# santi-pdp/segan_pytorch

Measured on AMD Instinct MI355X. Metric: 16384-sample waveform chunks/sec (GAN step), higher is better.
Workload: dtype f32

## Files before the change

segan_pytorch_amd/csrc/segan_conv.hip:

```cpp
#include "segan_conv_shared.h"

template <int MB, int NB, int WM, int U>
struct TileGeom {
  static constexpr int S = 32 / U;
  static constexpr int WN = 4 / WM;
  static constexpr int NI = MB / (32 * WM);
  static constexpr int NJ = NB / (32 * WN);
  static constexpr int NPT = MB / S;
};

struct TileWork {
  int tile, c0, c1;
  bool partial;
  int piece;
};

struct TileIter {
  int tileA;
  long unit, unit_end;
  int first_tile;
  __device__ __forceinline__ void init(const CorrArgs& a, int nch) {
    tileA = blockIdx.x;
    unit = (long)blockIdx.x * a.sk_units;
    unit_end = min(unit + (long)a.sk_units, a.sk_total);
// ... 293 lines not shown
            }
          }
        } else {
#pragma unroll
          for (int i = 0; i < NI; ++i) {
            const int rloc = 32 * (wm * NI + i) + (e & 3) + 8 * (e >> 2) + 4 * h;
            const int r = rloc / NPT;
            const int n = n0 + rloc % NPT;
            if (n >= a.Nout) continue;
            float v = acc[i][j][e] + (a.bias ? a.bias[n] : 0.0f);
            if (a.act == SEGAN_ACT_TANH) v = tanhf(v);
            const int P = S * q + r;
            int ii = P - a.o_padL;
            const size_t rowoff = (size_t)col_b[j] * a.Nout + n;
            if (ii >= 0 && ii < a.Lout) {
              if (a.o_roll != 0) {
                ii -= a.o_roll;
                if (ii < 0) ii += a.Lout;
                if (ii >= a.Lout) ii -= a.Lout;
              }
              a.out0[rowoff * (size_t)a.Lout + ii] = v;
            } else if (a.halo != nullptr) {
              if (ii < 0) a.halo[rowoff * hl + P] = v;
              else if (ii - a.Lout < a.o_padR) a.halo[rowoff * hl + a.o_padL + (ii - a.Lout)] = v;
            }
          }
        }
      }
    }
  }
}

template <int MB, bool OUT_HI>
__device__ __forceinline__ bool tile_is_dead(const CorrArgs& a, int m0) {
  if (OUT_HI) return false;
  if (a.out0 == nullptr && m0 + MB <= a.OC0) return true;
  if (a.out1 == nullptr && m0 >= a.OC0) return true;
  return false;
}

template <int MB, int U, int KC, int NI, int NJ, bool SHIFT, int FMODE = 0, int ZP = -1, int NPT = 32>
__device__ __forceinline__ void corr_mma_chunk(const float* Wl, const float* Il, int RLs,
                                               const int (&aoff)[NI], const int (&boff)[NJ],
                                               const int (&rsh)[NI], f32x16 (&acc)[NI][NJ],
                                               float (&b30)[NJ], int h, const int (&aoffx)[NI],
                                               const int (&boffx)[NJ]) {
  static_assert(FMODE == 0 || (!SHIFT && ZP < 0), "the pair trick of the F form has no row shifts");
  constexpr int NBI = SHIFT ? NI : 1;
  constexpr int CVC = KC / U;
  constexpr bool ZT = ZP >= 0 && CVC >= 2;
  typedef const volatile __attribute__((address_space(3))) float* ldsp;
  auto special = [](int i) { return ZT && (32 * i) / NPT == ZP; };
  auto skipped = [&](int i, int s) { return special(i) && ((2 * s) % U) == 0; };
  float av0[NI], av1[NI], bv0[NBI][NJ], bv1[NBI][NJ];
  auto read_step = [&](int s, float (&av)[NI], float (&bv)[NBI][NJ]) {
    const int kk = 2 * s;
    const int c = kk / U, u = kk % U;
    ldsp wr = (ldsp)(Wl + kk * MB);
    ldsp ir = (ldsp)(Il + c * RLs + u);
#pragma unroll
    for (int i = 0; i < NI; ++i)
      if (!skipped(i, s)) av[i] = wr[aoff[i]];
#pragma unroll
    for (int i = 0; i < NBI; ++i)
#pragma unroll
      for (int j = 0; j < NJ; ++j)
        if (!(SHIFT && skipped(i, s))) bv[i][j] = ir[boff[j] + (SHIFT ? rsh[i] : 0)];
  };
  constexpr int NS = FMODE == 1 ? KC / 2 - 1 : KC / 2;
  auto mma_step = [&](int s, const float (&av)[NI], float (&bv)[NBI][NJ]) {
    if (FMODE == 2 && s == NS - 1) {
#pragma unroll
      for (int j = 0; j < NJ; ++j) bv[0][j] = h ? b30[j] : bv[0][j];
    }
#pragma unroll
    for (int i = 0; i < NI; ++i)
#pragma unroll
      for (int j = 0; j < NJ; ++j)
        if (!skipped(i, s))
          acc[i][j] = __builtin_amdgcn_mfma_f32_32x32x2f32(av[i], bv[SHIFT ? i : 0][j], acc[i][j],
                                                           0, 0, 0);
  };
  if (FMODE == 1) {
    ldsp ir = (ldsp)(Il + (CVC - 1) * RLs + (U - 2));
#pragma unroll
    for (int j = 0; j < NJ; ++j) b30[j] = ir[boff[j] - h];
  }
  float avx[ZT ? CVC / 2 : 1][NI], bvx[ZT ? CVC / 2 : 1][NBI][NJ];
  if (ZT) {
#pragma unroll
    for (int p = 0; p < CVC / 2; ++p) {
      ldsp wr = (ldsp)(Wl + (2 * p * U + 1) * MB);
      ldsp ir = (ldsp)(Il + 2 * p * RLs + 1);
#pragma unroll
      for (int i = 0; i < NI; ++i)
        if (special(i)) avx[p][i] = wr[aoffx[i]];
#pragma unroll
      for (int i = 0; i < NBI; ++i)
#pragma unroll
        for (int j = 0; j < NJ; ++j)
          if (!SHIFT || special(i)) bvx[p][i][j] = ir[boffx[j] + (SHIFT ? rsh[i] : 0)];
    }
  }
  float av2[NI], bv2[NBI][NJ];
  read_step(0, av0, bv0);
  read_step(1, av1, bv1);
  if (ZT) {
    __builtin_amdgcn_sched_barrier(0);
#pragma unroll
    for (int p = 0; p < CVC / 2; ++p)
#pragma unroll
      for (int i = 0; i < NI; ++i)
#pragma unroll
        for (int j = 0; j < NJ; ++j)
          if (special(i))
            acc[i][j] = __builtin_amdgcn_mfma_f32_32x32x2f32(avx[p][i], bvx[p][SHIFT ? i : 0][j],
                                                             acc[i][j], 0, 0, 0);
  }
#pragma unroll
  for (int s = 0; s < NS; s += 3) {
    if (s + 2 < NS) read_step(s + 2, av2, bv2);
    __builtin_amdgcn_sched_barrier(0);
    mma_step(s, av0, bv0);
    __builtin_amdgcn_sched_barrier(0);
    if (s + 3 < NS) read_step(s + 3, av0, bv0);
    __builtin_amdgcn_sched_barrier(0);
    if (s + 1 < NS) mma_step(s + 1, av1, bv1);
    __builtin_amdgcn_sched_barrier(0);
    if (s + 4 < NS) read_step(s + 4, av1, bv1);
    __builtin_amdgcn_sched_barrier(0);
    if (s + 2 < NS) mma_step(s + 2, av2, bv2);
    __builtin_amdgcn_sched_barrier(0);
  }
}

template <int MB, int NB, int WM, int U, bool IN_HI, bool OUT_HI, bool SHIFT, int MAXPOS, int KC>
__global__ __launch_bounds__(256, 2) void corr_kernel(const CorrArgs a) {
  using G = TileGeom<MB, NB, WM, U>;
  constexpr int S = G::S, WN = G::WN, NI = G::NI, NJ = G::NJ, NPT = G::NPT;
  constexpr int SI = IN_HI ? S : 1;
  constexpr int CV = KC / U;
  static_assert(!OUT_HI || NPT % 32 == 0, "T-form tiles hold whole 32-row phase blocks");

  extern __shared__ __attribute__((aligned(16))) float smem[];
  const int RLs = a.RLs;
  float* Wl0 = smem;
  float* Il0 = smem + 2 * KC * MB;

  const int tid = threadIdx.x;
  const int lane = tid & 63;
  const int wave = __builtin_amdgcn_readfirstlane(tid >> 6);
  const int wm = wave / WN, wn = wave % WN;
  const int l31 = lane & 31, h = lane >> 5;

  const int nch = (a.Ktot + KC - 1) / KC;
  TileIter it;
  it.init(a, nch);
  TileWork tw;
  while (it.next(a, nch, tw)) {
  const int c0 = tw.c0, c1 = tw.c1;
  const int rowtile = a.rt0 + tw.tile / a.ncoltiles;
  const int coltile = tw.tile % a.ncoltiles;
  const int m0 = rowtile * MB;
  const int n0 = rowtile * NPT;
  if (tile_is_dead<MB, OUT_HI>(a, m0)) continue;
  const ColTile ct = make_coltile(coltile * NB, a.Tcols, NB);

  int pos_off[MAXPOS][SI];
  unsigned pos_ok[MAXPOS];
  int pos_bo0[MAXPOS], pos_bo1[MAXPOS];
#pragma unroll
  for (int pp = 0; pp < MAXPOS; ++pp) {
    const int j = tid + 256 * pp;
    pos_ok[pp] = 0u;
    pos_bo0[pp] = 0;
    pos_bo1[pp] = 0;
#pragma unroll
    for (int r = 0; r < SI; ++r) pos_off[pp][r] = 0;
    if (j < RLs) {
      int s, tau;
      lds_pos_decode(ct, j, a.Tcols, a.H, s, tau);
      const int b = ct.b0 + s;
      if (b < a.B) {
        pos_bo0[pp] = b * a.in.C0 * a.Lin;
        pos_bo1[pp] = b * a.in.C1 * a.Lin;
        const int wq = tau + a.win_start;
        if (IN_HI) {
#pragma unroll
          for (int r = 0; r < SI; ++r) {
            const int idx = segan_hi_index(S * wq + r, a.Lin, a.padL, a.mode, a.roll);
            if (idx >= 0) { pos_off[pp][r] = idx; pos_ok[pp] |= 1u << r; }
          }
        } else if (wq >= 0 && wq < a.Lin) {
          pos_off[pp][0] = wq;
          pos_ok[pp] = 1u;
        }
      }
    }
  }

  int aoff[NI], boff[NJ], rsh[NI];
#pragma unroll
  for (int i = 0; i < NI; ++i) {
    const int rloc = 32 * (wm * NI + i);
    aoff[i] = h * MB + rloc + l31;
    rsh[i] = SHIFT ? a.rowshift[rloc / NPT] : 0;
  }
  int col_b[NJ], col_t[NJ];
  lane_columns<NB, WN, NJ>(a, ct, wn, l31, h, col_b, col_t, boff);

  f32x16 acc[NI][NJ];
#pragma unroll
  for (int i = 0; i < NI; ++i)
#pragma unroll
    for (int j = 0; j < NJ; ++j)
#pragma unroll
      for (int e = 0; e < 16; ++e) acc[i][j][e] = 0.0f;

  constexpr int F4R = MB / 4;
  constexpr int RPP = 256 / F4R;
  constexpr int NPASS = KC / RPP;
  f32x4 wreg[NPASS];
  float ireg[CV][MAXPOS];
  const int wrow = tid / F4R, wc4 = tid % F4R;
  const int wgcol = OUT_HI ? ((4 * wc4) / NPT) * a.NP + n0 + (4 * wc4) % NPT : m0 + 4 * wc4;
  const float* wbase = a.wp + (size_t)wrow * a.RP + wgcol;

  auto load_chunk = [&](int ch) {
    const float* wsrc = wbase + (size_t)(ch * KC) * a.RP;
#pragma unroll
    for (int p = 0; p < NPASS; ++p)
      wreg[p] = *reinterpret_cast<const f32x4*>(wsrc + (size_t)(RPP * p) * a.RP);
#pragma unroll
    for (int c = 0; c < CV; ++c) {
      int cv = ch * CV + c;
      cv = cv < a.Cv ? cv : 0;
      const int n = IN_HI ? cv / S : cv;
      const int r = IN_HI ? c % S : 0;
      const bool seg1 = n >= a.in.C0;
      const float* rowp = seg1 ? a.in.p1 + (size_t)(n - a.in.C0) * a.Lin
                               : a.in.p0 + (size_t)n * a.Lin;
#pragma unroll
      for (int pp = 0; pp < MAXPOS; ++pp)
        ireg[c][pp] = rowp[(seg1 ? pos_bo1[pp] : pos_bo0[pp]) + pos_off[pp][r]];
    }
  };
  auto store_chunk = [&](int ch, int buf) {
    float* Wl = Wl0 + buf * (KC * MB);
    float* Il = Il0 + buf * (CV * RLs);
#pragma unroll
    for (int p = 0; p < NPASS; ++p) {
      if (IN_HI && a.f_pair && ((ch * KC + wrow + RPP * p) & 63) == 63)
        wreg[p] = f32x4{0.f, 0.f, 0.f, 0.f};
      *reinterpret_cast<f32x4*>(Wl + (wrow + RPP * p) * MB + 4 * wc4) = wreg[p];
    }
#pragma unroll
    for (int c = 0; c < CV; ++c) {
      const int cv = ch * CV + c;
      const bool cvalid = cv < a.Cv;
      const int n = IN_HI ? cv / S : cv;
      const int r = IN_HI ? c % S : 0;
      const ChanXf xf = segan_chan_xf(a.in, cvalid ? n : 0);
#pragma unroll
      for (int pp = 0; pp < MAXPOS; ++pp) {
        const int j = tid + 256 * pp;
        const bool ok = cvalid && ((pos_ok[pp] >> r) & 1u);
        const float v = ok ? segan_apply_xf(xf, ireg[c][pp]) : 0.0f;
        if (j < RLs) Il[c * RLs + j] = v;
      }
    }
  };

  float b30_unused[NJ] = {};
  load_chunk(c0);
  store_chunk(c0, 0);
  __syncthreads();
  for (int ch = c0; ch < c1; ++ch) {
    const int buf = (ch - c0) & 1;
    if (ch + 1 < c1) load_chunk(ch + 1);
    corr_mma_chunk<MB, U, KC, NI, NJ, SHIFT>(Wl0 + buf * (KC * MB), Il0 + buf * (CV * RLs), RLs,
                                             aoff, boff, rsh, acc, b30_unused, h, aoff, boff);
    if (ch + 1 < c1) store_chunk(ch + 1, buf ^ 1);
    __syncthreads();
  }

  if (tw.partial)
    slab_store<NI, NJ>(a.sk_ws + (size_t)(blockIdx.x * 2 + tw.piece) * (MB * NB), acc, tid);
  else
    corr_store_tile<MB, NB, WM, U, OUT_HI>(a, acc, m0, n0, wm, h, col_b, col_t);
  }
}

#define CORR2_KC 32
#define CORR2_NLD 4
template <int V>
struct IntC {
  static constexpr int value = V;
};

__device__ __forceinline__ float buf_load_f32(__amdgpu_buffer_rsrc_t r, int voff, int soff) {
  return __builtin_bit_cast(float, __builtin_amdgcn_raw_buffer_load_b32(r, voff, soff, 0));
}

template <int MB, int NB, int WM, int U, bool IN_HI, bool OUT_HI, bool SHIFT, bool XF, bool BLK = false>
__global__ __launch_bounds__(256, (IN_HI && !BLK) ? 4 : 2) void corr2_kernel(const CorrArgs a) {
  using G = TileGeom<MB, NB, WM, U>;
  constexpr int S = G::S, WN = G::WN, NI = G::NI, NJ = G::NJ, NPT = G::NPT;
  constexpr int KC = CORR2_KC;
  constexpr int CV = KC / U;
  constexpr int SL = 4 / CV;
  constexpr int NLD = CORR2_NLD;
  static_assert(CV == S, "one real channel per chunk of a HI input");
  static_assert(!OUT_HI || NPT % 32 == 0 || (!SHIFT && NPT % 4 == 0 && U != 8),
                "T-form tiles hold whole 32-row phase blocks");

  extern __shared__ __attribute__((aligned(16))) float smem[];
  const int RLs = a.RLs;
  float* Wl0 = smem;
  float* Il0 = smem + 2 * KC * MB;

  const int tid = threadIdx.x;
  const int lane = tid & 63;
  const int wave = __builtin_amdgcn_readfirstlane(tid >> 6);
  const int wm = wave / WN, wn = wave % WN;
  const int l31 = lane & 31, h = lane >> 5;
  const int wc = wave % CV;
  const int wslice = wave / CV;
  const int nld = a.nld;

  const __amdgpu_buffer_rsrc_t wrsrc =
      __builtin_amdgcn_make_buffer_rsrc(const_cast<float*>(a.wp), 0, 0x7fffffff, 0x00020000);
  constexpr int F4R = MB / 4;
  constexpr int RPI = 64 / F4R;
  constexpr int NINS = KC / RPI;
  constexpr int NPASS = NINS / 4;
  static_assert(NINS % 4 == 0, "weight tile instructions divide among 4 waves");

  const int nch = (a.Ktot + KC - 1) / KC;
  const int nchan = IN_HI ? a.Cv / S : a.Cv;
  TileIter it;
  it.init(a, nch);
  TileWork tw;
  while (it.next(a, nch, tw)) {
  const int c0 = tw.c0, c1 = tw.c1;
  const int rowtile = a.rt0 + tw.tile / a.ncoltiles;
  const int coltile = tw.tile % a.ncoltiles;
  const int m0 = rowtile * MB;
  const int n0 = rowtile * NPT;
  if (tile_is_dead<MB, OUT_HI>(a, m0)) continue;
  const ColTile ct = make_coltile(coltile * NB, a.Tcols, NB);

  const long left = (long)(a.B - ct.b0) * a.Lin * 4;
  const long nb0 = left * a.in.C0, nb1 = left * a.in.C1;
  const __amdgpu_buffer_rsrc_t r0 = __builtin_amdgcn_make_buffer_rsrc(
      const_cast<float*>(a.in.p0) + (size_t)ct.b0 * a.in.C0 * a.Lin, 0,
      (int)(nb0 < 0x7fffffffL ? nb0 : 0x7fffffffL), 0x00020000);
  const __amdgpu_buffer_rsrc_t r1 = __builtin_amdgcn_make_buffer_rsrc(
      a.in.C1 ? const_cast<float*>(a.in.p1) + (size_t)ct.b0 * a.in.C1 * a.Lin
              : const_cast<float*>(a.in.p0),
      0, (int)(nb1 < 0x7fffffffL ? nb1 : 0x7fffffffL), 0x00020000);

  int vo[NLD];
#pragma unroll
  for (int i = 0; i < NLD; ++i) {
    const int j = lane + 64 * (wslice + SL * i);
    vo[i] = (int)0x80000000u;
    if (i < nld && j < a.RLv) {
      int s, tau;
      lds_pos_decode(ct, j, a.Tcols, a.H, s, tau);
      if (ct.b0 + s < a.B) {
        const int wq = tau + a.win_start;
        int idx = -1;
        if (IN_HI) idx = segan_hi_index(S * wq + wc, a.Lin, a.padL, a.mode, a.roll);
        else if (wq >= 0 && wq < a.Lin) idx = wq;
        if (idx >= 0) vo[i] = (s * a.in.C0 * a.Lin + idx) * 4;
      }
    }
  }
  const int il_w = wc * RLs + lane + 64 * wslice;

  const int wrr = lane / F4R, wc4 = lane % F4R;
  const int wgcol = OUT_HI ? ((4 * wc4) / NPT) * a.NP + n0 + (4 * wc4) % NPT : m0 + 4 * wc4;
  const int wvo = (wrr * a.RP + wgcol) * 4;

  int aoff[NI], boff[NJ], rsh[NI];
#pragma unroll
  for (int i = 0; i < NI; ++i) {
    const int rloc = 32 * (wm * NI + i);
    aoff[i] = h * MB + rloc + l31;
    rsh[i] = SHIFT ? a.rowshift[rloc / NPT] : 0;
  }
  int col_b[NJ], col_t[NJ];
  lane_columns<NB, WN, NJ>(a, ct, wn, l31, h, col_b, col_t, boff);
  int aoffx[NI], boffx[NJ];
#pragma unroll
  for (int i = 0; i < NI; ++i) aoffx[i] = aoff[i] + h * (U - 1) * MB;
#pragma unroll
  for (int j = 0; j < NJ; ++j) boffx[j] = boff[j] + h * (RLs - 1);
  float b30[NJ];
#pragma unroll
  for (int j = 0; j < NJ; ++j) b30[j] = 0.0f;

  f32x16 acc[NI][NJ];
#pragma unroll
  for (int i = 0; i < NI; ++i)
#pragma unroll
    for (int j = 0; j < NJ; ++j)
#pragma unroll
      for (int e = 0; e < 16; ++e) acc[i][j][e] = 0.0f;

  f32x16 accs[BLK ? NI : 1][BLK ? NJ : 1];
  if (BLK) {
#pragma unroll
    for (int i = 0; i < NI; ++i)
#pragma unroll
      for (int j = 0; j < NJ; ++j)
#pragma unroll
        for (int e = 0; e < 16; ++e) accs[BLK ? i : 0][BLK ? j : 0][e] = 0.0f;
  }

  float ireg[NLD];
  float xsc = 1.0f, xsh = 0.0f, xsl = 1.0f;

  auto load_chunk = [&](int ch, int buf) {
    float* Wl = Wl0 + buf * (KC * MB);
#pragma unroll
    for (int p = 0; p < NPASS; ++p) {
      const int q = wave + 4 * p;
      __builtin_amdgcn_raw_ptr_buffer_load_lds(
          wrsrc, (__attribute__((address_space(3))) void*)(Wl + q * 256), 16, wvo,
          (ch * KC + q * RPI) * a.RP * 4, 0, 0);
    }
    const int chan = IN_HI ? ch : ch * CV + wc;
    const bool cok = chan < nchan;
    const bool seg1 = chan >= a.in.C0;
    const int cc = seg1 ? chan - a.in.C0 : chan;
    const int soff = cok ? cc * a.Lin * 4 : (int)0x7fffffff;
    if (XF) {
      typedef const __attribute__((address_space(4))) float* cptr;
      const int cx = cok ? chan : 0;
      xsl = ((cptr)a.in.slope)[cx];
      xsc = ((cptr)a.in.scale)[cx];
      xsh = ((cptr)a.in.shift)[cx];
    }
    const __amdgpu_buffer_rsrc_t rs = seg1 ? r1 : r0;
#pragma unroll
    for (int i = 0; i < NLD; ++i)
      if (i < nld) ireg[i] = buf_load_f32(rs, vo[i], soff);
  };
  auto store_chunk = [&](int buf) {
    float* Il = Il0 + buf * (CV * RLs) + il_w;
#pragma unroll
    for (int i = 0; i < NLD; ++i) {
      if (i < nld) {
        float v = ireg[i];
        if (XF) {
          v = fmaf(v, xsc, xsh);
          v = v > 0.0f ? v : v * xsl;
        }
        Il[64 * SL * i] = v;
      }
    }
  };

  load_chunk(c0, 0);
  store_chunk(0);
  __syncthreads();
  auto one_chunk = [&](auto fm, auto zp, int ch, auto sbuf) {
    int buf = decltype(sbuf)::value >= 0 ? decltype(sbuf)::value : (ch - c0) & 1;
    asm volatile("" : "+s"(buf));
    if (ch + 1 < c1) load_chunk(ch + 1, buf ^ 1);
    corr_mma_chunk<MB, U, KC, NI, NJ, SHIFT, decltype(fm)::value, decltype(zp)::value, NPT>(
        Wl0 + buf * (KC * MB), Il0 + buf * (CV * RLs), RLs, aoff, boff, rsh, acc, b30, h, aoffx, boffx);
    if (ch + 1 < c1) store_chunk(buf ^ 1);
    __syncthreads();
  };
  using Plain = IntC<0>;
  using NoZ = IntC<-1>;
  if constexpr (BLK) {
    static_assert(SEGAN_ACC_BLOCK % 2 == 0, "blocks hold whole channel pairs");
    for (int cb = c0; cb < c1; cb += SEGAN_ACC_BLOCK) {
      const int ce = min(cb + SEGAN_ACC_BLOCK, c1);
      if (IN_HI && a.f_pair) {
        for (int ch = cb; ch < ce; ch += 2) {
          one_chunk(IntC<(IN_HI && !SHIFT) ? 1 : 0>{}, NoZ{}, ch, NoZ{});
          one_chunk(IntC<(IN_HI && !SHIFT) ? 2 : 0>{}, NoZ{}, ch + 1, NoZ{});
        }
      } else {
        for (int ch = cb; ch < ce; ++ch) one_chunk(Plain{}, NoZ{}, ch, NoZ{});
      }
      acc_block_flush<NI, NJ>(acc, accs);
    }
  } else if constexpr (IN_HI && !SHIFT) {
    if (a.f_pair) {
      for (int ch = c0; ch < c1; ch += 2) {
        one_chunk(IntC<1>{}, NoZ{}, ch, IntC<0>{});
        one_chunk(IntC<2>{}, NoZ{}, ch + 1, IntC<1>{});
      }
    } else {
      for (int ch = c0; ch < c1; ++ch) one_chunk(Plain{}, NoZ{}, ch, NoZ{});
    }
  } else if constexpr (OUT_HI && U == 8) {
    constexpr int ZPK = SHIFT ? 2 : 3;
    if (a.zphase == ZPK) {
      for (int ch = c0; ch < c1; ++ch) one_chunk(Plain{}, IntC<ZPK>{}, ch, NoZ{});
    } else {
      for (int ch = c0; ch < c1; ++ch) one_chunk(Plain{}, NoZ{}, ch, NoZ{});
    }
  } else {
    for (int ch = c0; ch < c1; ++ch) one_chunk(Plain{}, NoZ{}, ch, NoZ{});
  }
  if constexpr (BLK) {
#pragma unroll
    for (int i = 0; i < NI; ++i)
#pragma unroll
      for (int j = 0; j < NJ; ++j) acc[i][j] = accs[i][j];
  }

  if (tw.partial)
    slab_store<NI, NJ>(a.sk_ws + (size_t)(blockIdx.x * 2 + tw.piece) * (MB * NB), acc, tid);
  else
    corr_store_tile<MB, NB, WM, U, OUT_HI>(a, acc, m0, n0, wm, h, col_b, col_t);
  }
}

template <int MB, int NB, int WM, int U, bool OUT_HI, int KC>
__global__ __launch_bounds__(256) void corr_fixup_kernel(const CorrArgs a) {
  using G = TileGeom<MB, NB, WM, U>;
  constexpr int WN = G::WN, NI = G::NI, NJ = G::NJ, NPT = G::NPT;
  const int tid = threadIdx.x;
  const int lane = tid & 63, wave = __builtin_amdgcn_readfirstlane(tid >> 6);
  const int wm = wave / WN, wn = wave % WN;
  const int l31 = lane & 31, h = lane >> 5;
  const int nch = (a.Ktot + KC - 1) / KC;
  const int t = blockIdx.x;
  const long u0 = (long)t * nch, u1 = u0 + nch - 1;
  const int g_first = (int)(u0 / a.sk_units), g_last = (int)(u1 / a.sk_units);
  if (g_first == g_last) return;
  const int tile = a.sk_nfull + t;
  const int rowtile = a.rt0 + tile / a.ncoltiles;
  const int coltile = tile % a.ncoltiles;
  const int m0 = rowtile * MB, n0 = rowtile * NPT;
  if (tile_is_dead<MB, OUT_HI>(a, m0)) return;
  const ColTile ct = make_coltile(coltile * NB, a.Tcols, NB);
  int col_b[NJ], col_t[NJ], boff[NJ];
  lane_columns<NB, WN, NJ>(a, ct, wn, l31, h, col_b, col_t, boff);
  f32x16 acc[NI][NJ];
#pragma unroll
  for (int i = 0; i < NI; ++i)
#pragma unroll
    for (int j = 0; j < NJ; ++j)
#pragma unroll
      for (int e = 0; e < 16; ++e) acc[i][j][e] = 0.0f;
  auto slab_of = [&](int g) {
    const int piece = t - (int)(((long)g * a.sk_units) / nch);
    return reinterpret_cast<const f32x4*>(a.sk_ws + (size_t)(g * 2 + piece) * (MB * NB));
  };
  constexpr int NV = NI * NJ * 4;
  for (int g = g_first; g <= g_last; g += 2) {
    const bool two = g + 1 <= g_last;
    const f32x4* s0 = slab_of(g);
    const f32x4* s1 = slab_of(two ? g + 1 : g);
    f32x4 v0[NV], v1[NV];
#pragma unroll
    for (int q = 0; q < NV; ++q) v0[q] = s0[q * 256 + tid];
    if (two) {
#pragma unroll
      for (int q = 0; q < NV; ++q) v1[q] = s1[q * 256 + tid];
    }
#pragma unroll
    for (int q = 0; q < NV; ++q)
#pragma unroll
      for (int e = 0; e < 4; ++e) acc[q / (NJ * 4)][(q / 4) % NJ][4 * (q % 4) + e] += v0[q][e];
    if (two) {
#pragma unroll
      for (int q = 0; q < NV; ++q)
#pragma unroll
        for (int e = 0; e < 4; ++e) acc[q / (NJ * 4)][(q / 4) % NJ][4 * (q % 4) + e] += v1[q][e];
    }
  }
  corr_store_tile<MB, NB, WM, U, OUT_HI>(a, acc, m0, n0, wm, h, col_b, col_t);
}

__global__ void fold_halo_kernel(float* dx, const float* halo, int rows, int L, int padL,
                                 int padR, int roll, int per_sample) {
  const int hl = padL + padR;
  if (per_sample) {
    const long t = (long)blockIdx.x * blockDim.x + threadIdx.x;
    if (t >= (long)rows * hl) return;
    const int row = (int)(t / hl), j = (int)(t - (long)row * hl);
    const int P = j < padL ? j : L + j;
    const int idx = segan_hi_index(P, L, padL, SEGAN_PAD_REFLECT, roll);
    if (idx >= 0) dx[(size_t)row * L + idx] += halo[(size_t)row * hl + j];
    return;
  }
  const int row = blockIdx.x * blockDim.x + threadIdx.x;
  if (row >= rows) return;
  float* d = dx + (size_t)row * L;
  const float* hrow = halo + (size_t)row * hl;
  for (int P = 0; P < padL; ++P) {
    const int idx = segan_hi_index(P, L, padL, SEGAN_PAD_REFLECT, roll);
    if (idx >= 0) d[idx] += hrow[P];
  }
  for (int P2 = 0; P2 < padR; ++P2) {
    const int idx = segan_hi_index(L + padL + P2, L, padL, SEGAN_PAD_REFLECT, roll);
    if (idx >= 0) d[idx] += hrow[padL + P2];
  }
}

#define CS_KC 16
struct ShortArgs {
  const float* da;
  const float* wg;
  float* dx;
  int B, N, M, L, Ls, padL, padRw, roll, ncoltiles;
  int xr8, xbc;
};

template <int S>
__global__ __launch_bounds__(256, 2) void conv_dgrad_short_kernel(const ShortArgs a) {
  constexpr int MB = 128, NB = 128, KC = CS_KC, NI = 2, NJ = 2, YP = 65, U = 32 / S;
  extern __shared__ __attribute__((aligned(16))) float smem[];
  float* Wl0 = smem;
  float* Il0 = smem + 2 * KC * MB;
  const int tid = threadIdx.x;
  const int lane = tid & 63;
  const int wave = __builtin_amdgcn_readfirstlane(tid >> 6);
  const int wm = wave >> 1, wn = wave & 1;
  const int l31 = lane & 31, h = lane >> 5;
  int rowtile, coltile;
  if (a.xbc > 0) {
    const int x = blockIdx.x & 7, k = blockIdx.x >> 3;
    const int per = a.xr8 * a.xbc;
    const int cb = k / per, rem = k - cb * per;
    const int wdt = min(a.xbc, a.ncoltiles - cb * a.xbc);
    const int rr = rem / wdt;
    rowtile = x * a.xr8 + rr;
    coltile = cb * a.xbc + rem - rr * wdt;
  } else {
    const int vb = xcd_remap(blockIdx.x, gridDim.x);
    rowtile = vb / a.ncoltiles;
    coltile = vb - rowtile * a.ncoltiles;
  }
  const int Ls = a.Ls, L = a.L;
  const int n0 = rowtile * 4;
  const int b0 = coltile * (NB / Ls);
  const int rowpitch = a.N * 32;

  const long wbytes = (long)a.M * rowpitch * 4, xbytes = (long)a.B * a.M * Ls * 4;
  const __amdgpu_buffer_rsrc_t wrs = __builtin_amdgcn_make_buffer_rsrc(
      const_cast<float*>(a.wg), 0, (int)(wbytes < 0x7fffffffL ? wbytes : 0x7fffffffL), 0x00020000);
  const __amdgpu_buffer_rsrc_t xrs = __builtin_amdgcn_make_buffer_rsrc(
      const_cast<float*>(a.da), 0, (int)(xbytes < 0x7fffffffL ? xbytes : 0x7fffffffL), 0x00020000);
  const int lr = lane >> 5, lc = 4 * (lane & 31);
  const int wvo = (lr * rowpitch + rowtile * MB + lc) * 4;
  const int s_l = lc / Ls, t_l = lc - s_l * Ls;
  const int xvo = (b0 + s_l < a.B) ? ((s_l * a.M + lr) * Ls + t_l) * 4 : (int)0x80000000u;

  auto load_chunk = [&](int ch, int buf) {
    float* Wl = Wl0 + buf * (KC * MB);
    float* Il = Il0 + buf * (KC * NB);
#pragma unroll
    for (int p = 0; p < KC / 8; ++p) {
      const int q = wave + 4 * p;
      __builtin_amdgcn_raw_ptr_buffer_load_lds(
          wrs, (__attribute__((address_space(3))) void*)(Wl + q * 256), 16, wvo,
          (ch * KC + 2 * q) * rowpitch * 4, 0, 0);
      __builtin_amdgcn_raw_ptr_buffer_load_lds(
          xrs, (__attribute__((address_space(3))) void*)(Il + q * 256), 16, xvo,
          ((b0 * a.M + ch * KC + 2 * q) * Ls) * 4, 0, 0);
    }
  };

  int aoff[NI], boff[NJ], rsh[NI];
#pragma unroll
  for (int i = 0; i < NI; ++i) {
    aoff[i] = h * MB + 32 * (wm * NI + i) + l31;
    rsh[i] = 0;
  }
#pragma unroll
  for (int j = 0; j < NJ; ++j) boff[j] = h * NB + 64 * wn + 32 * j + l31;

  f32x16 acc[NI][NJ];
#pragma unroll
  for (int i = 0; i < NI; ++i)
#pragma unroll
    for (int j = 0; j < NJ; ++j)
#pragma unroll
      for (int e = 0; e < 16; ++e) acc[i][j][e] = 0.0f;

  const int nch = a.M / KC;
  float b30_unused[NJ] = {};
  load_chunk(0, 0);
  __builtin_amdgcn_s_waitcnt(0x0f70);
  __syncthreads();
  for (int ch = 0; ch < nch; ++ch) {
    const int buf = ch & 1;
    if (ch + 1 < nch) load_chunk(ch + 1, buf ^ 1);
    corr_mma_chunk<MB, 1, KC, NI, NJ, false>(Wl0 + buf * (KC * MB), Il0 + buf * (KC * NB), NB, aoff,
                                             boff, rsh, acc, b30_unused, h, aoff, boff);
    __builtin_amdgcn_s_waitcnt(0x0f70);
    __syncthreads();
  }

  float* Yb = smem + wave * (32 * YP);
  const int bw = b0 + (64 * wn) / Ls;
  auto dxp = [&](int P, int cbase) -> float {
    const int r = P % S, qq = P / S;
    float v = 0.0f;
#pragma unroll
    for (int u = 0; u < U; ++u) {
      const int t = qq - u;
      if (t >= 0 && t < Ls) v += Yb[(r * U + u) * YP + cbase + t];
    }
    return v;
  };
#pragma unroll
  for (int i = 0; i < NI; ++i) {
#pragma unroll
    for (int j = 0; j < NJ; ++j)
#pragma unroll
      for (int e = 0; e < 16; ++e)
        Yb[((e & 3) + 8 * (e >> 2) + 4 * h) * YP + 32 * j + l31] = acc[i][j][e];
    __syncthreads();
    const int n = n0 + 2 * wm + i;
#pragma unroll
    for (int p = 0; p < S; ++p) {
      const int o = p * 64 + lane;
      const int sl = o / L, io = o - sl * L;
      const int b = bw + sl;
      float v = dxp(io + a.padL, sl * Ls);
      if (io >= 1 && io <= a.padL) v += dxp(a.padL - io, sl * Ls);
      const int jr = L - 2 - io;
      if (jr >= 0 && jr < a.padRw) v += dxp(L + a.padL + jr, sl * Ls);
      if (b < a.B && n < a.N) {
        int ii = io - a.roll;
        if (ii < 0) ii += L;
        if (ii >= L) ii -= L;
        a.dx[((size_t)b * a.N + n) * L + ii] = v;
      }
    }
    __syncthreads();
  }
}

__global__ void pack_g_kernel(const float* __restrict__ w, float* __restrict__ wg, int M, int N,
                              int K, int S) {
  const size_t total = (size_t)M * N * 32;
  const int U = 32 / S;
  for (size_t i = blockIdx.x * (size_t)blockDim.x + threadIdx.x; i < total;
       i += (size_t)gridDim.x * blockDim.x) {
    const int c = (int)(i & 31);
    const size_t mn = i >> 5;
    const int k = S * (c % U) + c / U;
    wg[i] = k < K ? w[mn * K + k] : 0.0f;
  }
}

static thread_local int g_last_corr[6];
void segan_note_corr_launch(int kind, unsigned grid, const CorrArgs& a, int ntiles) {
  g_last_corr[0] = kind;
  g_last_corr[1] = (int)grid;
  g_last_corr[2] = ntiles;
  g_last_corr[3] = a.sk_nfull;
  g_last_corr[4] = a.sk_total > 0 ? a.sk_units : 0;
  g_last_corr[5] = a.xf_mode;
}
extern "C" void segan_debug_last_corr(int* out6) {
  for (int i = 0; i < 6; ++i) out6[i] = g_last_corr[i];
}

static int cur_device() {
  int d = 0;
  (void)hipGetDevice(&d);
  return d & 15;
}

template <typename K>
static void allow_big_lds(K kern, bool (&done)[16]) {
  const int d = cur_device();
  if (!done[d]) {
    (void)hipFuncSetAttribute(reinterpret_cast<const void*>(kern),
                              hipFuncAttributeMaxDynamicSharedMemorySize, 160 * 1024);
    done[d] = true;
  }
}

template <typename K>
static int resident_per_cu(K kern, size_t lds, int (&occ)[16], size_t (&occ_lds)[16]) {
  const int d = cur_device();
  if (occ[d] == 0 || occ_lds[d] != lds) {
    int nb = 0;
    if (hipOccupancyMaxActiveBlocksPerMultiprocessor(&nb, reinterpret_cast<const void*>(kern), 256,
                                                     lds) != hipSuccess || nb < 1)
      nb = 2;
    occ[d] = nb > 4 ? 4 : nb;
    occ_lds[d] = lds;
  }
  return occ[d];
}

static unsigned plan_streamk(CorrArgs& a, int ntiles, int nch, int occ, size_t slab_floats,
                             bool allow, bool pair_cuts = false) {
  a.sk_nfull = ntiles;
  a.sk_units = 1;
  a.sk_total = 0;
  const double classic_eff = (double)ntiles / (256.0 * ceil_div(ntiles, 256));
  if (!allow || a.act != SEGAN_ACT_NONE || ntiles < 64 || nch < 8 || classic_eff >= 0.97) {
    if (allow && a.act == SEGAN_ACT_NONE && ntiles >= 2 * 256 * occ) return (unsigned)segan_grid_slots(occ);
    return (unsigned)ntiles;
  }
  const int G = segan_grid_slots(occ);
  if (a.sk_ws == nullptr || a.sk_ws_floats < (size_t)G * 2 * slab_floats) return (unsigned)ntiles;
  a.sk_nfull = (ntiles / G) * G;
  const int rem = ntiles - a.sk_nfull;
  if (rem == 0) return (unsigned)ntiles;
  a.sk_total = (long)rem * nch;
  a.sk_units = (int)((a.sk_total + G - 1) / G);
  if (pair_cuts) a.sk_units += a.sk_units & 1;
  return (unsigned)G;
}

template <int MB, int NB, int WM, int U, bool IN_HI, bool OUT_HI, bool SHIFT, int MAXPOS, int KC>
static int launch_corr_t(CorrArgs a, hipStream_t st, bool allow_sk) {
  constexpr int CV = KC / U;
  constexpr int S = 32 / U;
  const int nrowtiles = OUT_HI ? a.NP / (MB / S) : ceil_div(a.Rvalid, MB);
// ... 458 lines not shown
```

Baseline: 3571.

## Prefetch next tile's first chunk during last chunk of current tile

Restructures the persistent tile loop in corr2_kernel so that, on the last K-chunk of a tile, the block already fetches the next live tile and issues its first weight and input chunk loads into the other LDS buffer while the current MMA runs. Buffer parity is carried across tiles, and dead tiles are skipped inside the piece iterator. This hides the pipeline fill bubble at each tile boundary. In exchange, per-tile setup state becomes shared mutable state across tiles, which may raise register pressure. It also adds optional clock instrumentation that is off by default.

New measurement: 3397. -4.9%, worse.

```diff
diff --git a/segan_pytorch_amd/csrc/segan_conv.hip b/segan_pytorch_amd/csrc/segan_conv.hip
--- a/segan_pytorch_amd/csrc/segan_conv.hip
+++ b/segan_pytorch_amd/csrc/segan_conv.hip
@@ -619,6 +619,32 @@
   return __builtin_bit_cast(float, __builtin_amdgcn_raw_buffer_load_b32(r, voff, soff, 0));
 }
 
+#ifdef SEGAN_TILE_CLOCK
+#define SEGAN_TILE_CLOCK_VISITS 8
+#define SEGAN_TILE_CLOCK_WGS 8192
+#define SEGAN_TILE_CLOCK_ROW 8
+__device__ unsigned long long segan_tile_clock_buf[SEGAN_TILE_CLOCK_WGS * SEGAN_TILE_CLOCK_VISITS *
+                                                   SEGAN_TILE_CLOCK_ROW];
+#define CORR2_CLOCK(p)                                                                             \
+  do {                                                                                             \
+    if (tid == 0 && blockIdx.x < SEGAN_TILE_CLOCK_WGS && clk_visit < SEGAN_TILE_CLOCK_VISITS) {    \
+      unsigned long long* row_ = segan_tile_clock_buf +                                            \
+          ((size_t)blockIdx.x * SEGAN_TILE_CLOCK_VISITS + clk_visit) * SEGAN_TILE_CLOCK_ROW;       \
+      row_[p] = clock64();                                                                         \
+      if ((p) == 0) {                                                                              \
+        row_[4] = wall_clock64();                                                                  \
+        row_[5] = (unsigned long long)__builtin_amdgcn_s_getreg(63492) |                           \
+                  ((unsigned long long)__builtin_amdgcn_s_getreg(6164) << 32);                     \
+        row_[6] = (unsigned long long)(tw.c1 - tw.c0) | ((unsigned long long)tw.tile << 32);       \
+        row_[7] = 1;                                                                               \
+      }                                                                                            \
+    }                                                                                              \
+    if ((p) == 3) ++clk_visit;                                                                     \
+  } while (0)
+#else
+#define CORR2_CLOCK(p)
+#endif
+
 template <int MB, int NB, int WM, int U, bool IN_HI, bool OUT_HI, bool SHIFT, bool XF, bool BLK = false>
 __global__ __launch_bounds__(256, (IN_HI && !BLK) ? 4 : 2) void corr2_kernel(const CorrArgs a) {
   using G = TileGeom<MB, NB, WM, U>;
@@ -657,84 +683,50 @@
   const int nchan = IN_HI ? a.Cv / S : a.Cv;
   TileIter it;
   it.init(a, nch);
-  TileWork tw;
-  while (it.next(a, nch, tw)) {
-  const int c0 = tw.c0, c1 = tw.c1;
-  const int rowtile = a.rt0 + tw.tile / a.ncoltiles;
-  const int coltile = tw.tile % a.ncoltiles;
-  const int m0 = rowtile * MB;
-  const int n0 = rowtile * NPT;
-  if (tile_is_dead<MB, OUT_HI>(a, m0)) continue;
-  const ColTile ct = make_coltile(coltile * NB, a.Tcols, NB);
-
-  const long left = (long)(a.B - ct.b0) * a.Lin * 4;
-  const long nb0 = left * a.in.C0, nb1 = left * a.in.C1;
-  const __amdgpu_buffer_rsrc_t r0 = __builtin_amdgcn_make_buffer_rsrc(
-      const_cast<float*>(a.in.p0) + (size_t)ct.b0 * a.in.C0 * a.Lin, 0,
-      (int)(nb0 < 0x7fffffffL ? nb0 : 0x7fffffffL), 0x00020000);
-  const __amdgpu_buffer_rsrc_t r1 = __builtin_amdgcn_make_buffer_rsrc(
-      a.in.C1 ? const_cast<float*>(a.in.p1) + (size_t)ct.b0 * a.in.C1 * a.Lin
-              : const_cast<float*>(a.in.p0),
-      0, (int)(nb1 < 0x7fffffffL ? nb1 : 0x7fffffffL), 0x00020000);
-
+  auto next_piece = [&](TileWork& w) {
+    while (it.next(a, nch, w))
+      if (!tile_is_dead<MB, OUT_HI>(a, (a.rt0 + w.tile / a.ncoltiles) * MB)) return true;
+    return false;
+  };
+
+  __amdgpu_buffer_rsrc_t r0, r1;
   int vo[NLD];
-#pragma unroll
-  for (int i = 0; i < NLD; ++i) {
-    const int j = lane + 64 * (wslice + SL * i);
-    vo[i] = (int)0x80000000u;
-    if (i < nld && j < a.RLv) {
-      int s, tau;
-      lds_pos_decode(ct, j, a.Tcols, a.H, s, tau);
-      if (ct.b0 + s < a.B) {
-        const int wq = tau + a.win_start;
-        int idx = -1;
-        if (IN_HI) idx = segan_hi_index(S * wq + wc, a.Lin, a.padL, a.mode, a.roll);
-        else if (wq >= 0 && wq < a.Lin) idx = wq;
-        if (idx >= 0) vo[i] = (s * a.in.C0 * a.Lin + idx) * 4;
-      }
-    }
-  }
+  int wvo;
   const int il_w = wc * RLs + lane + 64 * wslice;
-
-  const int wrr = lane / F4R, wc4 = lane % F4R;
-  const int wgcol = OUT_HI ? ((4 * wc4) / NPT) * a.NP + n0 + (4 * wc4) % NPT : m0 + 4 * wc4;
-  const int wvo = (wrr * a.RP + wgcol) * 4;
-
-  int aoff[NI], boff[NJ], rsh[NI];
-#pragma unroll
-  for (int i = 0; i < NI; ++i) {
-    const int rloc = 32 * (wm * NI + i);
-    aoff[i] = h * MB + rloc + l31;
-    rsh[i] = SHIFT ? a.rowshift[rloc / NPT] : 0;
-  }
-  int col_b[NJ], col_t[NJ];
-  lane_columns<NB, WN, NJ>(a, ct, wn, l31, h, col_b, col_t, boff);
-  int aoffx[NI], boffx[NJ];
-#pragma unroll
-  for (int i = 0; i < NI; ++i) aoffx[i] = aoff[i] + h * (U - 1) * MB;
-#pragma unroll
-  for (int j = 0; j < NJ; ++j) boffx[j] = boff[j] + h * (RLs - 1);
-  float b30[NJ];
-#pragma unroll
-  for (int j = 0; j < NJ; ++j) b30[j] = 0.0f;
-
-  f32x16 acc[NI][NJ];
-#pragma unroll
-  for (int i = 0; i < NI; ++i)
-#pragma unroll
-    for (int j = 0; j < NJ; ++j)
-#pragma unroll
-      for (int e = 0; e < 16; ++e) acc[i][j][e] = 0.0f;
-
-  f32x16 accs[BLK ? NI : 1][BLK ? NJ : 1];
-  if (BLK) {
-#pragma unroll
-    for (int i = 0; i < NI; ++i)
-#pragma unroll
-      for (int j = 0; j < NJ; ++j)
-#pragma unroll
-        for (int e = 0; e < 16; ++e) accs[BLK ? i : 0][BLK ? j : 0][e] = 0.0f;
-  }
+  auto stage_setup = [&](const TileWork& w) {
+    const int rowtile = a.rt0 + w.tile / a.ncoltiles;
+    const int coltile = w.tile % a.ncoltiles;
+    const ColTile ct = make_coltile(coltile * NB, a.Tcols, NB);
+    const long left = (long)(a.B - ct.b0) * a.Lin * 4;
+    const long nb0 = left * a.in.C0, nb1 = left * a.in.C1;
+    r0 = __builtin_amdgcn_make_buffer_rsrc(
+        const_cast<float*>(a.in.p0) + (size_t)ct.b0 * a.in.C0 * a.Lin, 0,
+        (int)(nb0 < 0x7fffffffL ? nb0 : 0x7fffffffL), 0x00020000);
+    r1 = __builtin_amdgcn_make_buffer_rsrc(
+        a.in.C1 ? const_cast<float*>(a.in.p1) + (size_t)ct.b0 * a.in.C1 * a.Lin
+                : const_cast<float*>(a.in.p0),
+        0, (int)(nb1 < 0x7fffffffL ? nb1 : 0x7fffffffL), 0x00020000);
+#pragma unroll
+    for (int i = 0; i < NLD; ++i) {
+      const int j = lane + 64 * (wslice + SL * i);
+      vo[i] = (int)0x80000000u;
+      if (i < nld && j < a.RLv) {
+        int s, tau;
+        lds_pos_decode(ct, j, a.Tcols, a.H, s, tau);
+        if (ct.b0 + s < a.B) {
+          const int wq = tau + a.win_start;
+          int idx = -1;
+          if (IN_HI) idx = segan_hi_index(S * wq + wc, a.Lin, a.padL, a.mode, a.roll);
+          else if (wq >= 0 && wq < a.Lin) idx = wq;
+          if (idx >= 0) vo[i] = (s * a.in.C0 * a.Lin + idx) * 4;
+        }
+      }
+    }
+    const int wrr = lane / F4R, wc4 = lane % F4R;
+    const int wgcol = OUT_HI ? ((4 * wc4) / NPT) * a.NP + rowtile * NPT + (4 * wc4) % NPT
+                             : rowtile * MB + 4 * wc4;
+    wvo = (wrr * a.RP + wgcol) * 4;
+  };
 
   float ireg[NLD];
   float xsc = 1.0f, xsh = 0.0f, xsl = 1.0f;
@@ -780,16 +772,82 @@
     }
   };
 
-  load_chunk(c0, 0);
-  store_chunk(0);
-  __syncthreads();
+  TileWork tw, twn;
+  bool have = next_piece(tw);
+  if (have) {
+    stage_setup(tw);
+    load_chunk(tw.c0, 0);
+    store_chunk(0);
+    __syncthreads();
+  }
+  int pb = 0;
+#ifdef SEGAN_TILE_CLOCK
+  int clk_visit = 0;
+#endif
+  while (have) {
+  CORR2_CLOCK(0);
+  const int c0 = tw.c0, c1 = tw.c1;
+  const int rowtile = a.rt0 + tw.tile / a.ncoltiles;
+  const int coltile = tw.tile % a.ncoltiles;
+  const int m0 = rowtile * MB;
+  const int n0 = rowtile * NPT;
+  const ColTile ct = make_coltile(coltile * NB, a.Tcols, NB);
+  bool have_next = false;
+
+  int aoff[NI], boff[NJ], rsh[NI];
+#pragma unroll
+  for (int i = 0; i < NI; ++i) {
+    const int rloc = 32 * (wm * NI + i);
+    aoff[i] = h * MB + rloc + l31;
+    rsh[i] = SHIFT ? a.rowshift[rloc / NPT] : 0;
+  }
+  int col_b[NJ], col_t[NJ];
+  lane_columns<NB, WN, NJ>(a, ct, wn, l31, h, col_b, col_t, boff);
+  int aoffx[NI], boffx[NJ];
+#pragma unroll
+  for (int i = 0; i < NI; ++i) aoffx[i] = aoff[i] + h * (U - 1) * MB;
+#pragma unroll
+  for (int j = 0; j < NJ; ++j) boffx[j] = boff[j] + h * (RLs - 1);
+  float b30[NJ];
+#pragma unroll
+  for (int j = 0; j < NJ; ++j) b30[j] = 0.0f;
+
+  f32x16 acc[NI][NJ];
+#pragma unroll
+  for (int i = 0; i < NI; ++i)
+#pragma unroll
+    for (int j = 0; j < NJ; ++j)
+#pragma unroll
+      for (int e = 0; e < 16; ++e) acc[i][j][e] = 0.0f;
+
+  f32x16 accs[BLK ? NI : 1][BLK ? NJ : 1];
+  if (BLK) {
+#pragma unroll
+    for (int i = 0; i < NI; ++i)
+#pragma unroll
+      for (int j = 0; j < NJ; ++j)
+#pragma unroll
+        for (int e = 0; e < 16; ++e) accs[BLK ? i : 0][BLK ? j : 0][e] = 0.0f;
+  }
+
+  CORR2_CLOCK(1);
   auto one_chunk = [&](auto fm, auto zp, int ch, auto sbuf) {
-    int buf = decltype(sbuf)::value >= 0 ? decltype(sbuf)::value : (ch - c0) & 1;
+    int buf = decltype(sbuf)::value >= 0 ? decltype(sbuf)::value : (ch - c0 + pb) & 1;
     asm volatile("" : "+s"(buf));
-    if (ch + 1 < c1) load_chunk(ch + 1, buf ^ 1);
+    bool staged = true;
+    if (ch + 1 < c1) {
+      load_chunk(ch + 1, buf ^ 1);
+    } else if (decltype(fm)::value != 1) {
+      have_next = next_piece(twn);
+      if (have_next) {
+        stage_setup(twn);
+        load_chunk(twn.c0, buf ^ 1);
+      }
+      staged = have_next;
+    }
     corr_mma_chunk<MB, U, KC, NI, NJ, SHIFT, decltype(fm)::value, decltype(zp)::value, NPT>(
         Wl0 + buf * (KC * MB), Il0 + buf * (CV * RLs), RLs, aoff, boff, rsh, acc, b30, h, aoffx, boffx);
-    if (ch + 1 < c1) store_chunk(buf ^ 1);
+    if (staged) store_chunk(buf ^ 1);
     __syncthreads();
   };
   using Plain = IntC<0>;
@@ -834,12 +892,30 @@
       for (int j = 0; j < NJ; ++j) acc[i][j] = accs[i][j];
   }
 
+  CORR2_CLOCK(2);
   if (tw.partial)
     slab_store<NI, NJ>(a.sk_ws + (size_t)(blockIdx.x * 2 + tw.piece) * (MB * NB), acc, tid);
   else
     corr_store_tile<MB, NB, WM, U, OUT_HI>(a, acc, m0, n0, wm, h, col_b, col_t);
-  }
-}
+  CORR2_CLOCK(3);
+  pb = (pb + c1 - c0) & 1;
+  tw = twn;
+  have = have_next;
+  }
+}
+
+#ifdef SEGAN_TILE_CLOCK
+extern "C" int segan_tile_clock_read(unsigned long long* host, size_t n) {
+  const size_t all = sizeof(segan_tile_clock_buf) / sizeof(unsigned long long);
+  if (n > all) n = all;
+  if (hipDeviceSynchronize() != hipSuccess) return SEGAN_ELAUNCH;
+  if (hipMemcpyFromSymbol(host, HIP_SYMBOL(segan_tile_clock_buf), n * 8) != hipSuccess) return SEGAN_ELAUNCH;
+  void* dp = nullptr;
+  if (hipGetSymbolAddress(&dp, HIP_SYMBOL(segan_tile_clock_buf)) != hipSuccess) return SEGAN_ELAUNCH;
+  if (hipMemset(dp, 0, sizeof(segan_tile_clock_buf)) != hipSuccess) return SEGAN_ELAUNCH;
+  return SEGAN_OK;
+}
+#endif
 
 template <int MB, int NB, int WM, int U, bool OUT_HI, int KC>
 __global__ __launch_bounds__(256) void corr_fixup_kernel(const CorrArgs a) {
```
